# nihui/realsr-ncnn-vulkan

Measured on AMD Instinct MI355X. Metric: output Mpix/s (4x upscale) DF2K tile=200, higher is better.
Workload: dtype f16

## Files before the change

### realsr-ncnn-vulkan_amd/csrc/conv_flow.hip

```cpp
#include "kernels.h"
#include "model.h"

namespace rsr {

typedef _Float16 half8 __attribute__((ext_vector_type(8)));
typedef _Float16 half4 __attribute__((ext_vector_type(4)));
typedef _Float16 half2v __attribute__((ext_vector_type(2)));
typedef float f32x16 __attribute__((ext_vector_type(16)));
typedef unsigned int u32x4 __attribute__((ext_vector_type(4)));
typedef unsigned int u32x2 __attribute__((ext_vector_type(2)));
typedef int i32x8 __attribute__((ext_vector_type(8)));
typedef float f32x4 __attribute__((ext_vector_type(4)));
typedef float f32x2 __attribute__((ext_vector_type(2)));
typedef f32x4 __attribute__((may_alias)) f32x4_lds;

namespace {

constexpr int kFPx = 32;
constexpr int kFRow = kPatchW * kFPx;
constexpr int kFPatch = 20 * 1024;
constexpr int kFPieces = 20;
constexpr int kFItems = kPatchPx * 2;

template <int NT>
struct FlowCfg
{
    static constexpr int PR = NT == 1 ? 6 : 4;
#ifndef RSR_STREAM_WR
#define RSR_STREAM_WR 3
#endif
    static constexpr int WR = RSR_STREAM_WR;
    static constexpr int WB = NT * 9 * 32 * 32;
    static constexpr int WPIECES = NT * 9;
    static constexpr int W_OFF = PR * kFPatch;
    static constexpr int BIAS_OFF = W_OFF + WR * WB;
    static constexpr int TOTAL = BIAS_OFF + NT * 128;
};
static_assert(FlowCfg<1>::TOTAL <= 160 * 1024 && FlowCfg<2>::TOTAL <= 160 * 1024, "LDS budget");

__device__ __forceinline__ const char* plane_ptr(const PlaneSrc& s, int slot, int plane)
{
    return static_cast<const char*>(s.base) + (long long)slot * s.slot_stride + (long long)plane * s.plane_stride;
}

__device__ __forceinline__ WorkItem load_item(const WorkItem* items, int idx)
{
    typedef const __attribute__((address_space(4))) i32x8* cptr_t;
    const i32x8 v = *(cptr_t)(unsigned long long)(items + idx);
    WorkItem it;
    it.slot = __builtin_amdgcn_readfirstlane(v[0]);
    it.y0 = __builtin_amdgcn_readfirstlane(v[1]);
    it.x0 = __builtin_amdgcn_readfirstlane(v[2]);
    it.H = __builtin_amdgcn_readfirstlane(v[3]);
    it.W = __builtin_amdgcn_readfirstlane(v[4]);
    it.pad0 = __builtin_amdgcn_readfirstlane(v[5]);
    it.pad1 = __builtin_amdgcn_readfirstlane(v[6]);
    it.pad2 = __builtin_amdgcn_readfirstlane(v[7]);
    return it;
}

__device__ __forceinline__ char* uniform_ptr(const void* p)
{
    const unsigned long long b = (unsigned long long)p;
    const unsigned lo = (unsigned)__builtin_amdgcn_readfirstlane((int)(unsigned)b);
    const unsigned hi = (unsigned)__builtin_amdgcn_readfirstlane((int)(unsigned)(b >> 32));
    return reinterpret_cast<char*>((unsigned long long)lo | ((unsigned long long)hi << 32));
}

__device__ __forceinline__ f32x2 bf8_pair(unsigned w, int hiword)
{
    return hiword ? __builtin_amdgcn_cvt_pk_f32_bf8(int(w), true) : __builtin_amdgcn_cvt_pk_f32_bf8(int(w), false);
}
__device__ __forceinline__ int pack_bf8_pair(float x, float y, int old, int hiword)
{
    return hiword ? __builtin_amdgcn_cvt_pk_bf8_f32(x, y, old, true) : __builtin_amdgcn_cvt_pk_bf8_f32(x, y, old, false);
}

#define RSR_LDS(p) ((__attribute__((address_space(3))) void*)(p))
#define RSR_GLB(p) ((const __attribute__((address_space(1))) void*)(p))
#define RSR_MFMA 0x8
#define RSR_DSR 0x100
#define RSR_SG(mask, n) __builtin_amdgcn_sched_group_barrier(mask, n, 0)

#ifdef RSR_EXPERIMENT
#define RSR_ABL(bits) (a.dbg & (bits))
#else
#define RSR_ABL(bits) 0
#if defined(RSR_FLOW_LIFE) || defined(RSR_FLOW_TRACE) || defined(RSR_EXP_THIN)
#error "RSR_FLOW_LIFE / RSR_FLOW_TRACE / RSR_EXP_THIN are experiment builds: add -DRSR_EXPERIMENT"
#endif
#endif

}

template <int NT, int NTW, bool UPS, int EPI, bool DEFER, bool WRES>
__global__ __launch_bounds__((4 * NT / NTW + 4) * 64, (4 * NT / NTW + 4) / 4) void conv3x3_flow(const ConvArgs a)
{
    extern __shared__ __attribute__((aligned(16))) char smem[];
    typedef FlowCfg<NT> C;
    constexpr int MW = 4 * NT / NTW;
    constexpr int WB = C::WB;
    constexpr bool WDB = (NTW == 1);
    static_assert(!DEFER || (NT == 1 && NTW == 1), "deferred epilogue needs the 256-VGPR budget of the 8-wave workgroup");
    constexpr bool LAST3 = (EPI == 3 || EPI == 6 || EPI == 8 || EPI == 9);
    constexpr bool LASTG = (EPI == 0 || EPI == 7 || EPI == 10 || EPI == 11);
    constexpr bool OUT32 = (EPI == 6 || EPI == 7 || EPI == 9 || EPI == 11);
    constexpr bool FIMG = EPI >= 8;
    static_assert(!LAST3 || (NT == 1 && NTW == 1 && !UPS && !DEFER && WRES), "conv_last's (dy, cout) layout: 32 rows, resident aux image");
    static_assert((EPI != 4 && EPI != 5) || (NT == 2 && NTW == 1 && !UPS && !DEFER), "the precise residual epilogue exists for the 64-output-channel convs of the trunk");
    constexpr bool RESID = (EPI == 2 || EPI == 4 || EPI == 5);
    constexpr bool PREC = (EPI == 4 || EPI == 5);

    const int tid = threadIdx.x;
    const int lane = tid & 63;
    const int wave = __builtin_amdgcn_readfirstlane(tid >> 6);
#ifdef RSR_FLOW_LIFE
    const unsigned long long life_t0 = __builtin_amdgcn_s_memtime();
#define RSR_LIFE(SLOT) if (a.trace && tid == 0) a.trace[blockIdx.x * 4 + (SLOT)] = __builtin_amdgcn_s_memtime();
#else
#define RSR_LIFE(SLOT)
#endif
    const int nst = a.n0 + a.n1;
    const int PR = WRES ? a.pr : C::PR, WR = WRES ? nst : C::WR;
    const int kWOff = PR * kFPatch, kBiasOff = kWOff + WR * (LAST3 ? a.wpieces * 1024 : WB);

    const int per = (a.nitems + 7) >> 3;
    const int xcd = blockIdx.x & 7, j = blockIdx.x >> 3, nj = gridDim.x >> 3;
    const int first = xcd * per + j;
    const int end = min((xcd + 1) * per, a.nitems);
    const int nmine = first < end ? (end - first + nj - 1) / nj : 0;
    if (nmine == 0) return;
    const int S = nmine * nst;

    if (tid < NT * 32) reinterpret_cast<float*>(smem + kBiasOff)[tid] = a.bias[tid];
    __syncthreads();

    if (wave >= MW)
    {
        const int lw = wave - MW;
        constexpr int NP = kFPieces / 4;
        const int nW = (C::WPIECES - lw + 3) / 4;
        int pr[NP], pc[NP], pxor[NP];
        bool pvalid[NP];
#pragma unroll
        for (int i = 0; i < NP; i++)
        {
            const int jj = (lw + 4 * i) * 64 + lane;
            const int px = jj >> 1;
            pr[i] = px / kPatchW;
            pc[i] = px - pr[i] * kPatchW;
            pxor[i] = ((jj & 1) ^ ((pc[i] >> 3) & 1)) << 4;
            pvalid[i] = jj < kFItems;
        }
        const char* wsrc_lane = static_cast<const char*>(a.wpk16) + lw * 1024 + lane * 16;

        int uP = 0, uW = 0, sP = 0, sW = 0, ckP = 0, ckW = 0, rP = 0;
        WorkItem itP = load_item(a.items, first);
        unsigned srcoff[NP];
        auto block_offsets = [&]() {
            const int H = itP.H, W = itP.W, Wi = UPS ? (W >> 1) : W;
            const bool fold = (itP.x0 & kFoldBit) != 0;
            const int bx0 = itP.x0 & (kFoldBit - 1);
#pragma unroll
            for (int i = 0; i < NP; i++)
            {
                const int half = (fold && pc[i] >= 16) ? 16 : 0;
                const int gy = itP.y0 - 1 + pr[i] + half, gx = bx0 - 1 + pc[i] - half;
                const bool ok = pvalid[i] && gy >= 0 && gy < H && gx >= 0 && gx < W;
                const int sy = UPS ? (gy >> 1) : gy, sx = UPS ? (gx >> 1) : gx;
                srcoff[i] = ok ? unsigned(kGuard + (sy * Wi + sx) * kFPx + pxor[i]) : 0u;
            }
        };
        block_offsets();
        auto issueP = [&]() {
            if (uP >= S) return;
            const char* gbase = ((ckP < a.n0) ? plane_ptr(a.src0, itP.slot, ckP) : plane_ptr(a.src1, itP.slot, ckP - a.n0)) - kGuard;
            char* dst = smem + sP * kFPatch + lw * 1024;
            if (!RSR_ABL(1 | 128))
            {
#pragma unroll
                for (int i = 0; i < NP; i++)
                    __builtin_amdgcn_global_load_lds(RSR_GLB(gbase + srcoff[i]), RSR_LDS(dst + i * 4096), 16, 0, 0);
            }
            sP = sP == PR - 1 ? 0 : sP + 1;
            uP++;
            if (++ckP == nst)
            {
                ckP = 0;
                if (++rP < nmine)
                {
                    itP = load_item(a.items, first + rP * nj);
                    block_offsets();
                }
            }
        };
        auto issueW = [&]() {
            if (uW >= S) return;
            const char* src = wsrc_lane + (long long)ckW * WB;
            char* dst = smem + kWOff + sW * WB + lw * 1024;
            if (!RSR_ABL(1 | 64))
            {
#pragma unroll
                for (int i = 0; i < (C::WPIECES + 3) / 4; i++)
                    if (i < nW)
                        __builtin_amdgcn_global_load_lds(RSR_GLB(src + i * 4096), RSR_LDS(dst + i * 4096), 16, 0, 0);
            }
            sW = sW == WR - 1 ? 0 : sW + 1;
            uW++;
            ckW = ckW + 1 == nst ? 0 : ckW + 1;
        };
        if (WRES)
        {
            const int npieces = nst * (LAST3 ? a.wpieces : C::WPIECES);
            if (!RSR_ABL(1 | 64))
                for (int p_ = lw; p_ < npieces; p_ += 4)
                    __builtin_amdgcn_global_load_lds(RSR_GLB(static_cast<const char*>(a.wpk16) + p_ * 1024 + lane * 16), RSR_LDS(smem + kWOff + p_ * 1024), 16, 0, 0);
            for (int tt = -(PR - 1); tt < 0; tt++) issueP();
            for (int t = 0; t < S; t++)
            {
                if (RSR_ABL(1) || t + PR - 2 >= S) asm volatile("s_waitcnt vmcnt(0)\n\ts_barrier" ::: "memory");
                else if (PR == 3) asm volatile("s_waitcnt vmcnt(%0)\n\ts_barrier" ::"n"(1 * NP) : "memory");
                else if (PR == 4) asm volatile("s_waitcnt vmcnt(%0)\n\ts_barrier" ::"n"(2 * NP) : "memory");
                else if (PR == 5) asm volatile("s_waitcnt vmcnt(%0)\n\ts_barrier" ::"n"(3 * NP) : "memory");
                else if (PR == 6) asm volatile("s_waitcnt vmcnt(%0)\n\ts_barrier" ::"n"(4 * NP) : "memory");
                else asm volatile("s_waitcnt vmcnt(0)\n\ts_barrier" ::: "memory");
                issueP();
            }
        }
        else
        {
            for (int tt = -(PR - 1); tt < 0; tt++)
            {
                if (tt + WR - 1 >= 0) issueW();
                issueP();
            }
            constexpr int WRm2 = C::WR - 2;
            constexpr int NW_HI = (C::WPIECES + 3) / 4, NW_LO = C::WPIECES / 4;
            for (int t = 0; t < S; t++)
            {
                if (RSR_ABL(1) || t + PR - 2 >= S) asm volatile("s_waitcnt vmcnt(0)\n\ts_barrier" ::: "memory");
                else if (RSR_ABL(64)) asm volatile("s_waitcnt vmcnt(%0)\n\ts_barrier" ::"n"((WRm2 + 1) * NP) : "memory");
                else if (RSR_ABL(128) && nW == NW_HI) asm volatile("s_waitcnt vmcnt(%0)\n\ts_barrier" ::"n"(WRm2 * NW_HI) : "memory");
                else if (RSR_ABL(128)) asm volatile("s_waitcnt vmcnt(%0)\n\ts_barrier" ::"n"(WRm2 * NW_LO) : "memory");
                else if (nW == NW_HI) asm volatile("s_waitcnt vmcnt(%0)\n\ts_barrier" ::"n"((WRm2 + 1) * NP + WRm2 * NW_HI) : "memory");
                else asm volatile("s_waitcnt vmcnt(%0)\n\ts_barrier" ::"n"((WRm2 + 1) * NP + WRm2 * NW_LO) : "memory");
                issueW();
                issueP();
            }
        }
        asm volatile("s_barrier" ::: "memory");
        return;
    }

    const int l32 = lane & 31, hi = lane >> 5;
    const int wrow = wave & 3, ntw0 = (wave >> 2) * NTW;
    int xcol[3];
#pragma unroll
    for (int dx = 0; dx < 3; dx++)
    {
        const int c = l32 + dx;
        xcol[dx] = wrow * 4 * kFRow + c * kFPx + ((hi ^ ((c >> 3) & 1)) << 4);
    }
    const int woff = kWOff + (ntw0 * 32 + l32) * 32 + ((hi ^ ((l32 >> 3) & 1)) << 4);

    f32x16 bias16[NTW];
    auto load_bias = [&]() {
#pragma unroll
        for (int n = 0; n < NTW; n++)
#pragma unroll
            for (int q = 0; q < 4; q++)
            {
                const f32x4 b4 = *reinterpret_cast<const f32x4_lds*>(smem + kBiasOff + ((ntw0 + n) * 32 + q * 8 + hi * 4) * 4);
#pragma unroll
                for (int e = 0; e < 4; e++) bias16[n][q * 4 + e] = b4[e];
            }
    };
    load_bias();

    const float slope = a.lrelu ? 0.2f : 1.f;
    const bool idt = RESID && a.res1_in_acc;
    const bool has2 = EPI == 5 || ((EPI == 2) && a.res2_kind == 1);
#ifdef RSR_FLOW_TRACE
    const bool tracing = a.trace && blockIdx.x == 0 && wave == 0;
#else
    constexpr bool tracing = false;
#endif

    float pinf0 = __builtin_inff();
    asm volatile("" : "+s"(pinf0));

    struct OutDesc
    {
        char* base;
        int live;
        int voff;
        int y0, H, W, slot;
        unsigned lim;
    };
    auto make_out = [&](const WorkItem& it, bool live) {
        OutDesc o;
        o.base = const_cast<char*>(plane_ptr(a.out16, it.slot, ntw0 * 2));
        o.live = (live && !RSR_ABL(4)) ? 1 : 0;
        const bool fold = (it.x0 & kFoldBit) != 0;
        const int x = (it.x0 & (kFoldBit - 1)) + (fold ? (l32 & 15) : l32);
        o.voff = x < it.W ? x * kFPx + hi * 16 + ((fold && l32 >= 16) ? 16 * it.W * kFPx : 0) : int(0x80000000u);
        o.y0 = it.y0 + wrow * 4;
        o.H = it.H;
        o.W = it.W;
        o.slot = it.slot;
        o.lim = unsigned(it.H) * unsigned(it.W * kFPx);
        return o;
    };
    auto row_pack = [&](const f32x16& acc, u32x4 (&tq)[2]) {
#pragma unroll
        for (int p = 0; p < 2; p++)
        {
            half8 o;
#pragma unroll
            for (int e = 0; e < 8; e++)
            {
                float v = acc[p * 8 + e];
                if (EPI == 2)
                {
                    v = v * a.s1;
                    asm volatile("" : "+v"(v));
                }
                else v = __builtin_amdgcn_fmed3f(v, v * slope, pinf0);
                o[e] = (_Float16)v;
            }
            tq[p] = __builtin_bit_cast(u32x4, o);
        }
    };
    constexpr bool PRE2 = (EPI == 2 || EPI == 4) && NTW == 1;
    u32x4 r2q[PRE2 ? 2 : 1][NTW][2];
#ifndef RSR_PREC_PRE
#define RSR_PREC_PRE 1
#endif
    u32x4 l1q[EPI == 4 ? 4 : 1];
    auto res2_row = [&](u32x4 (&dst)[2], const OutDesc& o, int rr, int n) {
        const int y = o.y0 + rr;
        char* ub = uniform_ptr(const_cast<char*>(plane_ptr(a.res2, o.slot, ntw0 * 2)));
        const unsigned pstride = unsigned(a.res2.plane_stride);
#pragma unroll
        for (int p = 0; p < 2; p++)
        {
            const unsigned poff = unsigned(n * 2 + p) * pstride;
            const __amdgpu_buffer_rsrc_t rs = __builtin_amdgcn_make_buffer_rsrc(ub, 0, int(o.lim + poff), 0x00020000);
            dst[p] = __builtin_amdgcn_raw_buffer_load_b128(rs, o.voff, int(unsigned(y) * unsigned(o.W * kFPx) + poff), 0);
        }
    };
    auto lo_row = [&](const PlaneSrc& s, long long off, u32x4& dst, const OutDesc& o, int rr, int n) {
        const int y = o.y0 + rr;
        const unsigned pstride = unsigned(s.plane_stride);
        char* ub = uniform_ptr(const_cast<char*>(plane_ptr(s, o.slot, 0)) + off + (long long)(ntw0 + n) * pstride);
        const __amdgpu_buffer_rsrc_t rs = __builtin_amdgcn_make_buffer_rsrc(ub, 0, off ? int(o.lim) : 0, 0x00020000);
        dst = __builtin_amdgcn_raw_buffer_load_b128(rs, o.voff, int(unsigned(y) * unsigned(o.W * kFPx)), 0);
    };
    auto res2_prefetch = [&](const WorkItem& w, int row0) {
        if (!PRE2) return;
        if (EPI == 4)
        {
            if (row0 != 0) return;
            const OutDesc o = make_out(w, true);
#pragma unroll
            for (int rr = 0; rr < RSR_PREC_PRE; rr++) lo_row(a.res1, a.lo1_off, l1q[EPI == 4 ? rr : 0], o, rr, 0);
            __builtin_amdgcn_sched_barrier(0);
            return;
        }
        if (!has2) return;
        const OutDesc o = make_out(w, true);
#pragma unroll
        for (int rr = 0; rr < 2; rr++)
#pragma unroll
            for (int n = 0; n < NTW; n++) res2_row(r2q[PRE2 ? rr : 0][n], o, row0 + rr, n);
        __builtin_amdgcn_sched_barrier(0);
    };
    auto row_store = [&](const u32x4 (&tq)[2], const OutDesc& o, int rr, int n) {
        const int y = o.y0 + rr;
        char* ub = uniform_ptr(o.base);
        const unsigned pstride = unsigned(a.out16.plane_stride);
#pragma unroll
        for (int p = 0; p < 2; p++)
        {
            const unsigned poff = unsigned(n * 2 + p) * pstride;
            const __amdgpu_buffer_rsrc_t rs = __builtin_amdgcn_make_buffer_rsrc(ub, 0, o.live ? int(o.lim + poff) : 0, 0x00020000);
            __builtin_amdgcn_raw_buffer_store_b128(tq[p], rs, o.voff + int(unsigned(y) * unsigned(o.W * kFPx) + poff), 0, 0);
        }
    };
    auto row_emit = [&](const f32x16& acc, const OutDesc& o, int rr, int n) {
        const int y = o.y0 + rr;
        char* ub = uniform_ptr(o.base);
        const unsigned pstride = unsigned(a.out16.plane_stride);
        u32x4 r2x[2];
        if (EPI == 2 && has2 && !PRE2) res2_row(r2x, o, rr, n);
#pragma unroll
        for (int p = 0; p < 2; p++)
        {
            half8 v;
#pragma unroll
            for (int e = 0; e < 8; e++)
            {
                float f = acc[p * 8 + e];
                if (EPI == 2)
                {
                    f = f * a.s1;
                    asm volatile("" : "+v"(f));
                }
                else f = __builtin_amdgcn_fmed3f(f, f * slope, pinf0);
                v[e] = (_Float16)f;
            }
            if (EPI == 2 && has2)
            {
                const half8 r2 = __builtin_bit_cast(half8, PRE2 ? r2q[PRE2 ? (rr & 1) : 0][n][p] : r2x[p]);
#pragma unroll
                for (int e = 0; e < 8; e++)
                {
                    float f = __builtin_fmaf((float)v[e], a.s2, (float)r2[e]);
                    asm volatile("" : "+v"(f));
                    v[e] = (_Float16)f;
                }
            }
            const unsigned poff = unsigned(n * 2 + p) * pstride;
            const __amdgpu_buffer_rsrc_t rs = __builtin_amdgcn_make_buffer_rsrc(ub, 0, o.live ? int(o.lim + poff) : 0, 0x00020000);
            __builtin_amdgcn_raw_buffer_store_b128(__builtin_bit_cast(u32x4, v), rs, o.voff + int(unsigned(y) * unsigned(o.W * kFPx) + poff), 0, 0);
            __builtin_amdgcn_sched_barrier(0);
        }
    };
    constexpr float kLoScale = 2048.f, kLoInv = 1.f / 2048.f;
    auto row_emit4 = [&](const f32x16& acc, const OutDesc& o, int rr, int n, const u32x4& l1, const u32x4 (&r2h)[2], const u32x4& r2l) {
        const int y = o.y0 + rr;
        char* ub = uniform_ptr(o.base);
        const unsigned pstride = unsigned(a.out16.plane_stride);
        char* ul = uniform_ptr(const_cast<char*>(plane_ptr(a.out16, o.slot, 0)) + a.out_lo_off + (long long)(ntw0 + n) * pstride);
        const unsigned rowoff = unsigned(y) * unsigned(o.W * kFPx);
        u32x4 vl;
#pragma unroll
        for (int p = 0; p < 2; p++)
        {
            half8 vh;
            const half8 r = __builtin_bit_cast(half8, r2h[p]);
#pragma unroll
            for (int k = 0; k < 2; k++)
            {
                int wq = 0;
#pragma unroll
                for (int e2 = 0; e2 < 2; e2++)
                {
                    const int c0 = p * 8 + k * 4 + e2 * 2;
                    const f32x2 av = {acc[c0], acc[c0 + 1]};
                    const f32x2 kinv = {kLoInv, kLoInv}, s1v = {a.s1, a.s1};
                    f32x2 f = __builtin_elementwise_fma(bf8_pair(l1[p * 2 + k], e2), kinv, av * s1v);
                    if (EPI == 5)
                    {
                        const f32x2 rv = {(float)r[k * 4 + e2 * 2], (float)r[k * 4 + e2 * 2 + 1]}, s2v = {a.s2, a.s2};
                        f = __builtin_elementwise_fma(bf8_pair(r2l[p * 2 + k], e2), kinv, __builtin_elementwise_fma(f, s2v, rv));
                    }
                    asm volatile("" : "+v"(f));
                    const half2v hv = __builtin_convertvector(f, half2v);
                    vh[k * 4 + e2 * 2] = hv[0];
                    vh[k * 4 + e2 * 2 + 1] = hv[1];
                    const f32x2 ksc = {kLoScale, kLoScale};
                    const f32x2 t = (f - __builtin_convertvector(hv, f32x2)) * ksc;
                    wq = pack_bf8_pair(t[0], t[1], wq, e2);
                }
                vl[p * 2 + k] = unsigned(wq);
            }
            const unsigned poff = unsigned(n * 2 + p) * pstride;
            const __amdgpu_buffer_rsrc_t rs = __builtin_amdgcn_make_buffer_rsrc(ub, 0, o.live ? int(o.lim + poff) : 0, 0x00020000);
            __builtin_amdgcn_raw_buffer_store_b128(__builtin_bit_cast(u32x4, vh), rs, o.voff + int(rowoff + poff), 0, 0);
            __builtin_amdgcn_sched_barrier(0);
        }
        const __amdgpu_buffer_rsrc_t rl = __builtin_amdgcn_make_buffer_rsrc(ul, 0, (o.live && a.out_lo_off) ? int(o.lim) : 0, 0x00020000);
        __builtin_amdgcn_raw_buffer_store_b128(vl, rl, o.voff + int(rowoff), 0, 0);
        __builtin_amdgcn_sched_barrier(0);
    };
    auto store3 = [&](const float (&val)[4][3], const WorkItem& it) {
        if (hi != 0 || ntw0 != 0 || RSR_ABL(4)) return;
        const bool fold = (it.x0 & kFoldBit) != 0;
        const int x = (it.x0 & (kFoldBit - 1)) + (fold ? (l32 & 15) : l32);
        const int yb = it.y0 + wrow * 4 + ((fold && l32 >= 16) ? 16 : 0);
        if (a.out_u8)
        {
            const int ox = it.pad0 + x, ow = pad2_w(it.pad2), oh = pad2_h(it.pad2);
            const int oim = pad2_img(it.pad2);
            uint8_t* const oimg = a.out_u8s[oim];
            const int opitch = a.out_pitch[oim];
            if constexpr (FIMG)
            {
                const long long cstep = a.out_plane[oim];
                const int esh = a.out_fmt == kFmtF32 ? 2 : 1;
#pragma unroll
                for (int rr = 0; rr < 4; rr++)
                {
                    const int y = yb + rr;
                    const int rx = x - a.out_u8_crop, ry = y - a.out_u8_crop;
                    if (rx >= 0 && rx < ow && ry >= 0 && ry < oh)
                    {
                        const long long pix = (long long)(it.pad1 + y) * opitch + ((long long)ox << esh);
#pragma unroll
                        for (int ch = 0; ch < 3; ch++)
                        {
                            float v = OUT32 ? val[rr][ch] : (float)(_Float16)val[rr][ch];
                            v = fminf(fmaxf(v, 0.f), 1.f);
                            uint8_t* const e = oimg + (a.out_u8_bgr ? 2 - ch : ch) * cstep + pix;
                            if (a.out_fmt == kFmtF32) *reinterpret_cast<float*>(e) = v;
                            else *reinterpret_cast<_Float16*>(e) = (_Float16)v;
                        }
                    }
                }
                return;
            }
#pragma unroll
            for (int rr = 0; rr < 4; rr++)
            {
                const int y = yb + rr;
                const int rx = x - a.out_u8_crop, ry = y - a.out_u8_crop;
                if (rx >= 0 && rx < ow && ry >= 0 && ry < oh)
                {
                    uint8_t* o = oimg + (long long)(it.pad1 + y) * opitch + ox * 3;
#pragma unroll
                    for (int ch = 0; ch < 3; ch++)
                    {
                        float v = OUT32 ? val[rr][ch] : (float)(_Float16)val[rr][ch];
                        v = floorf(v * 255.f + 0.5f);
                        v = fminf(fmaxf(v, 0.f), 255.f);
                        o[a.out_u8_bgr ? 2 - ch : ch] = (uint8_t)v;
                    }
                }
            }
            return;
        }
        _Float16* o = reinterpret_cast<_Float16*>(static_cast<char*>(a.out_planar3) + (long long)it.slot * a.planar3_slot_stride);
        const long long hw = (long long)it.H * it.W;
#pragma unroll
        for (int rr = 0; rr < 4; rr++)
        {
            const int y = yb + rr;
            if (y < it.H && x < it.W)
            {
                const long long pix = (long long)y * it.W + x;
#pragma unroll
                for (int ch = 0; ch < 3; ch++)
                {
                    float v = val[rr][ch];
                    if (a.lrelu) v = fmaxf(v, v * 0.2f);
                    if (OUT32) reinterpret_cast<float*>(o)[ch * hw + pix] = v;
                    else o[ch * hw + pix] = (_Float16)v;
                }
            }
        }
    };
    auto planar_store = [&](const f32x16 (&acc)[4][NTW], const WorkItem& it) {
        float val[4][3];
#pragma unroll
        for (int rr = 0; rr < 4; rr++)
#pragma unroll
            for (int ch = 0; ch < 3; ch++) val[rr][ch] = acc[rr][0][ch];
        store3(val, it);
    };

    half8 X[6], Wa[3][NTW], Wb[WDB ? 3 : 1][NTW];
    f32x16 accA[4][NTW], accB[DEFER ? 4 : 1][NTW];

    int sP = 0, sW = 0;
    int r = 0, ck = 0, t = 0;
    auto xbase = [&](int slot, int dx) { return smem + slot * kFPatch + xcol[dx]; };
    auto wbase = [&](int slot) { return smem + slot * WB + woff; };
#define RSR_LDX(R, XB) X[R] = *reinterpret_cast<const half8*>((XB) + (R)*kFRow);
#define RSR_LDW(WS, DY, DX, WBASE)                                                                                   \
    _Pragma("unroll") for (int n_ = 0; n_ < NTW; n_++) WS[DY][n_] =                                                  \
        *reinterpret_cast<const half8*>((WBASE) + ((DY)*3 + (DX)) * (NT * 1024) + n_ * 1024);
#ifndef RSR_EXP_THIN
#define RSR_CELL(ACC, WS, DY, RR, FIRST)                                                                             \
    _Pragma("unroll") for (int n_ = 0; n_ < NTW; n_++) ACC[RR][n_] = __builtin_amdgcn_mfma_f32_32x32x16_f16(         \
        WS[DY][n_], X[(RR) + (DY)], ((FIRST) && (DY) == 0) ? bias16[n_] : ACC[RR][n_], 0, 0, 0);
#else
#define RSR_KEEP(DY, RR)                                                                                             \
    ((DY) == 0 || (RSR_EXP_THIN == 24 && (DY) == 1) ||                                                               \
     (RSR_EXP_THIN == 16 && ((curdx_ == 0 && (DY) == 1 && (RR) == 0) || (curdx_ == 1 && (DY) == 1 && (RR) == 1) || (curdx_ == 2 && (DY) == 2 && (RR) < 2))))
#define RSR_CELL(ACC, WS, DY, RR, FIRST)                                                                             \
    if (RSR_KEEP(DY, RR))                                                                                            \
    {                                                                                                                \
        _Pragma("unroll") for (int n_ = 0; n_ < NTW; n_++) ACC[RR][n_] = __builtin_amdgcn_mfma_f32_32x32x16_f16(     \
            WS[DY][n_], X[(RR) + (DY)], ((FIRST) && (DY) == 0) ? bias16[n_] : ACC[RR][n_], 0, 0, 0);                 \
        if (RSR_EXP_THIN == 16 || ((DY) == 0 && (RR) < 3))                                                           \
        {                                                                                                            \
            half8 y_ = X[((RR) + (DY)) % 6] + X[((RR) + 2 * (DY) + 1) % 6];          \
            if (RSR_EXP_THIN == 16) y_ = y_ + X[((RR) + (DY) + 3) % 6];                                              \
            asm volatile("" ::"v"(y_));                                                                              \
        }                                                                                                            \
    }
#endif
#define RSR_NOHK(c)

#define RSR_STEP(ACC, WCUR, WNXT, NXB, NWB, NDX, FIRST, BAR, ITEMQ, HK)                                              \
    {                                                                                                                \
        constexpr int curdx_ = ((NDX) + 2) % 3;                 \
        (void)curdx_;                                                                                                \
        if ((BAR) && (ITEMQ))                                                                        \
        {                                                                                                            \
            const WorkItem* ip_ = a.items + (first + min(r + 2, nmine - 1) * nj);                                    \
            asm volatile("s_load_dwordx8 %0, %1, 0x0" : "=s"(item_q) : "s"(ip_));                                    \
        }                                                                                                            \
        RSR_CELL(ACC, WCUR, 0, 0, FIRST) HK(0)                                                                       \
        if (!(BAR)) { RSR_LDX(0, NXB) if (WDB) { RSR_LDW(WNXT, 0, NDX, NWB) } }                                      \
        RSR_CELL(ACC, WCUR, 0, 1, FIRST) HK(1) RSR_CELL(ACC, WCUR, 1, 0, FIRST) HK(2)                                \
        if (BAR)                                                                                                     \
        {                                                                                                            \
            __builtin_amdgcn_sched_barrier(0);                                                                       \
            if (tracing) t_arr = __builtin_amdgcn_s_memtime();                                                       \
            if (ITEMQ) asm volatile("s_waitcnt lgkmcnt(0)\n\ts_barrier" : "+s"(item_q)::"memory");                   \
            else asm volatile("s_waitcnt lgkmcnt(0)\n\ts_barrier" ::: "memory");                                     \
            if (tracing) t_rel = __builtin_amdgcn_s_memtime();                                                       \
            __builtin_amdgcn_sched_barrier(0);                                                                       \
            RSR_LDX(0, NXB) if (WDB) { RSR_LDW(WNXT, 0, NDX, NWB) }                                                  \
        }                                                                                                            \
        RSR_LDX(1, NXB) if (WDB) { RSR_LDW(WNXT, 1, NDX, NWB) }                                                      \
        RSR_CELL(ACC, WCUR, 1, 1, FIRST) HK(3) RSR_CELL(ACC, WCUR, 2, 0, FIRST) HK(4) RSR_CELL(ACC, WCUR, 2, 1, FIRST) HK(5) \
        if (WDB) { RSR_LDW(WNXT, 2, NDX, NWB) }                                                                      \
        RSR_CELL(ACC, WCUR, 0, 2, FIRST) HK(6)                                                                       \
        RSR_LDX(2, NXB)                                                                                              \
        RSR_CELL(ACC, WCUR, 0, 3, FIRST) HK(7)                                                                       \
        if (!WDB) { RSR_LDW(WNXT, 0, NDX, NWB) }                                                                     \
        RSR_CELL(ACC, WCUR, 1, 2, FIRST) HK(8)                                                                       \
        RSR_LDX(3, NXB)                                                                                              \
        RSR_CELL(ACC, WCUR, 1, 3, FIRST) HK(9)                                                                       \
        if (!WDB) { RSR_LDW(WNXT, 1, NDX, NWB) }                                                                     \
        RSR_CELL(ACC, WCUR, 2, 2, FIRST) HK(10)                                                                      \
        RSR_LDX(4, NXB)                                                                                              \
        RSR_CELL(ACC, WCUR, 2, 3, FIRST) HK(11)                                                                      \
        RSR_LDX(5, NXB)                                                                                              \
        if (!WDB) { RSR_LDW(WNXT, 2, NDX, NWB) }                                                                     \
    }
#define RSR_STEP_SCHED(BAR, PIN)                                                                                     \
    if (PIN)                                                                                                         \
    {                                                                                                                \
        if (BAR)                                                                                                     \
        {                                                                                                            \
            RSR_SG(RSR_DSR, WDB ? 4 : 2);                                                                            \
            RSR_SG(RSR_MFMA, 3 * NTW);                                                                               \
        }                                                                                                            \
        else                                                                                                         \
        {                                                                                                            \
            RSR_SG(RSR_MFMA, 1 * NTW); RSR_SG(RSR_DSR, WDB ? 2 : 1);                                                 \
            RSR_SG(RSR_MFMA, 2 * NTW); RSR_SG(RSR_DSR, WDB ? 2 : 1);                                                 \
            RSR_SG(RSR_MFMA, 3 * NTW);                                                                               \
        }                                                                                                            \
        if (WDB)                                                                                                     \
        {                                                                                                            \
            RSR_SG(RSR_DSR, 1);                                                                                      \
            RSR_SG(RSR_MFMA, 1); RSR_SG(RSR_DSR, 1);                                                                 \
            RSR_SG(RSR_MFMA, 2); RSR_SG(RSR_DSR, 1);                                                                 \
            RSR_SG(RSR_MFMA, 2); RSR_SG(RSR_DSR, 1);                                                                 \
            RSR_SG(RSR_MFMA, 1); RSR_SG(RSR_DSR, 1);                                                                 \
        }                                                                                                            \
        else                                                                                                         \
        {                                                                                                            \
            RSR_SG(RSR_MFMA, 1 * NTW); RSR_SG(RSR_DSR, 1);                                                           \
            RSR_SG(RSR_MFMA, 1 * NTW); RSR_SG(RSR_DSR, NTW);                                                         \
            RSR_SG(RSR_MFMA, 1 * NTW); RSR_SG(RSR_DSR, 1);                                                           \
            RSR_SG(RSR_MFMA, 1 * NTW); RSR_SG(RSR_DSR, NTW);                                                         \
            RSR_SG(RSR_MFMA, 1 * NTW); RSR_SG(RSR_DSR, 1);                                                           \
            RSR_SG(RSR_MFMA, 1 * NTW); RSR_SG(RSR_DSR, 1 + NTW);                                                     \
        }                                                                                                            \
    }
#define RSR_IDTAP(ACC)                                                                                               \
    if (RESID && idt)                                                                                                \
    {                                                                                                                \
        __builtin_amdgcn_sched_barrier(0);                                                                           \
        _Pragma("unroll") for (int n_ = 0; n_ < NTW; n_++) if ((ck >> 1) == ntw0 + n_)                               \
        {                                                                                                            \
            half8 idf;                                                                                               \
            int l32i = l32;                                                                                          \
            if (PREC) asm volatile("" : "+v"(l32i));  \
            _Pragma("unroll") for (int e = 0; e < 8; e++) idf[e] =                                                   \
                ((ck & 1) * 16 + hi * 8 + e == row_cout(l32i)) ? (_Float16)a.res1_coef : (_Float16)0.f;              \
            const char* cb_ = xbase(sP, 1);                                                                          \
            _Pragma("unroll") for (int rr = 0; rr < 4; rr++)                                                         \
            {                                                                                                        \
                const half8 xc = *reinterpret_cast<const half8*>(cb_ + (rr + 1) * kFRow);                            \
                ACC[rr][n_] = __builtin_amdgcn_mfma_f32_32x32x16_f16(idf, xc, ACC[rr][n_], 0, 0, 0);                 \
            }                                                                                                        \
        }                                                                                                            \
        __builtin_amdgcn_sched_barrier(0);                                                                           \
    }
#define RSR_HALF(ACC, W0, W1, FIRST, HK0, P0, HK1, P1, HK2, P2)                                                      \
    {                                                                                                                \
        const int nsP = sP == PR - 1 ? 0 : sP + 1, nsW = sW == WR - 1 ? 0 : sW + 1;                                  \
        {                                                                                                            \
            const char* nxb = xbase(sP, 1);                                                                          \
            const char* nwb = wbase(sW);                                                                             \
            RSR_STEP(ACC, W0, W1, nxb, nwb, 1, FIRST, false, false, HK0)                                             \
            RSR_STEP_SCHED(false, P0)                                                                                \
        }                                                                                                            \
        RSR_IDTAP(ACC)                                                                                               \
        {                                                                                                            \
            const char* nxb = xbase(sP, 2);                                                                          \
            const char* nwb = wbase(sW);                                                                             \
            RSR_STEP(ACC, W1, W0, nxb, nwb, 2, false, false, false, HK1)                                             \
            RSR_STEP_SCHED(false, P1)                                                                                \
        }                                                                                                            \
        {                                                                                                            \
            const char* nxb = xbase(nsP, 0);                                                                         \
            const char* nwb = wbase(nsW);                                                                            \
            RSR_STEP(ACC, W0, W1, nxb, nwb, 0, false, true, FIRST, HK2)                                              \
            RSR_STEP_SCHED(true, P2)                                                                                 \
        }                                                                                                            \
        if (tracing && lane == 0 && t + 1 < 512)                                                                     \
        {                                                                                                            \
            a.trace[2 * (t + 1)] = t_arr;                                                                            \
            a.trace[2 * (t + 1) + 1] = t_rel;                                                                        \
        }                                                                                                            \
        sP = nsP;                                                                                                    \
        sW = nsW;                                                                                                    \
        t++;                                                                                                         \
    }
#define RSR_HALF_PLAIN(ACC, W0, W1, FIRST) RSR_HALF(ACC, W0, W1, FIRST, RSR_NOHK, 1, RSR_NOHK, 1, RSR_NOHK, 1)

    WorkItem it = load_item(a.items, first);
    WorkItem nxt = load_item(a.items, first + (nmine > 1 ? nj : 0));
    i32x8 item_q = {0, 0, 0, 0, 0, 0, 0, 0};
    auto item_from_q = [&]() {
        WorkItem w;
        w.slot = item_q[0]; w.y0 = item_q[1]; w.x0 = item_q[2]; w.H = item_q[3]; w.W = item_q[4];
        w.pad0 = item_q[5]; w.pad1 = item_q[6]; w.pad2 = item_q[7];
        return w;
    };

    auto wave_is_dead = [&](const WorkItem& w) {
        const int y = w.y0 + wrow * 4;
        return (y >= w.H - a.margin || y + 4 <= a.margin) && !(a.dbg & 32);
    };
    auto skip_block = [&]() {
        {
            const WorkItem* ip_ = a.items + (first + min(r + 2, nmine - 1) * nj);
            asm volatile("s_load_dwordx8 %0, %1, 0x0" : "=s"(item_q) : "s"(ip_));
        }
        for (int h_ = 0; h_ < nst; h_++)
        {
            asm volatile("s_waitcnt lgkmcnt(0)\n\ts_barrier" : "+s"(item_q)::"memory");
            sP = sP == PR - 1 ? 0 : sP + 1;
            sW = sW == WR - 1 ? 0 : sW + 1;
            t++;
        }
        __builtin_amdgcn_sched_barrier(0);
        const char* xb = xbase(sP, 0);
        const char* wb = wbase(sW);
#pragma unroll
        for (int q = 0; q < 6; q++) { RSR_LDX(q, xb) }
#pragma unroll
        for (int dy = 0; dy < 3; dy++) { RSR_LDW(Wa, dy, 0, wb) }
        if (!DEFER) load_bias();
        __builtin_amdgcn_sched_barrier(0);
    };

    unsigned long long t_arr = 0, t_rel = 0;
    (void)t_rel;
    if (tracing) t_arr = __builtin_amdgcn_s_memtime();
    asm volatile("s_barrier" ::: "memory");
#ifdef RSR_FLOW_LIFE
    if (a.trace && tid == 0) a.trace[blockIdx.x * 4 + 0] = life_t0;
    RSR_LIFE(1)
#endif
    if (tracing && lane == 0)
    {
        a.trace[0] = t_arr;
        a.trace[1] = __builtin_amdgcn_s_memtime();
    }
    if constexpr (LAST3)
    {
        f32x16 acc[6];
        half8 Xa[6], Xb[6], Wfa, Wfb;
        const int woff3 = kWOff + l32 * 32 + ((hi ^ ((l32 >> 3) & 1)) << 4);
        const int WB3 = a.wpieces * 1024;
        auto ldx = [&](half8(&Xf)[6], int slot, int dx) {
            const char* xb = xbase(slot, dx);
#pragma unroll
            for (int q = 0; q < 6; q++) Xf[q] = *reinterpret_cast<const half8*>(xb + q * kFRow);
        };
        auto ldw = [&](int plane, int dx) { return *reinterpret_cast<const half8*>(smem + woff3 + plane * WB3 + dx * 1024); };
        const f32x16 zero16 = {0.f, 0.f, 0.f, 0.f, 0.f, 0.f, 0.f, 0.f, 0.f, 0.f, 0.f, 0.f, 0.f, 0.f, 0.f, 0.f};
#define RSR_M6(XF, WF, FIRST)                                                                                        \
    _Pragma("unroll") for (int q = 0; q < 6; q++) acc[q] = __builtin_amdgcn_mfma_f32_32x32x16_f16(WF, XF[q], (FIRST) ? zero16 : acc[q], 0, 0, 0);
#define RSR_HALF3(XC, WC, XN, WN, FIRST)                                                                             \
    {                                                                                                                \
        const int nsP = sP == PR - 1 ? 0 : sP + 1, nck = ck + 1 == nst ? 0 : ck + 1;                                 \
        if (FIRST)  \
        {                                                                                                            \
            const WorkItem* ip_ = a.items + (first + min(r + 2, nmine - 1) * nj);                                    \
            asm volatile("s_load_dwordx8 %0, %1, 0x0" : "=s"(item_q) : "s"(ip_));                                    \
        }                                                                                                            \
        ldx(XN, sP, 1); WN = ldw(ck, 1);                                                                             \
        RSR_M6(XC, WC, FIRST)                                                                                        \
        ldx(XC, sP, 2); WC = ldw(ck, 2);                                                                             \
        RSR_M6(XN, WN, false)                                                                                        \
        __builtin_amdgcn_sched_barrier(0);                                                                           \
        asm volatile("s_waitcnt lgkmcnt(0)\n\ts_barrier" : "+s"(item_q)::"memory");                                  \
        __builtin_amdgcn_sched_barrier(0);                                                                           \
        ldx(XN, nsP, 0); WN = ldw(nck, 0);                                                                           \
        RSR_M6(XC, WC, false)                                                                                        \
        sP = nsP;                                                                                                    \
        t++;                                                                                                         \
    }
        ldx(Xa, 0, 0);
        Wfa = ldw(0, 0);
        for (r = 0; r < nmine; r++)
        {
            while (wave_is_dead(it))
            {
                {
                    const WorkItem* ip_ = a.items + (first + min(r + 2, nmine - 1) * nj);
                    asm volatile("s_load_dwordx8 %0, %1, 0x0" : "=s"(item_q) : "s"(ip_));
                }
                for (int h_ = 0; h_ < nst; h_++)
                {
                    asm volatile("s_waitcnt lgkmcnt(0)\n\ts_barrier" : "+s"(item_q)::"memory");
                    sP = sP == PR - 1 ? 0 : sP + 1;
                    t++;
                }
                ldx(Xa, sP, 0);
                Wfa = ldw(0, 0);
                it = nxt;
                nxt = item_from_q();
                if (++r >= nmine) break;
            }
            if (r >= nmine) break;
            for (int cp = 0; cp < nst; cp += 2)
            {
                ck = cp;
                if (cp == 0) { RSR_HALF3(Xa, Wfa, Xb, Wfb, true) }
                else { RSR_HALF3(Xa, Wfa, Xb, Wfb, false) }
                ck = cp + 1;
                RSR_HALF3(Xb, Wfb, Xa, Wfa, false)
            }
            __builtin_amdgcn_sched_barrier(0);
            float val[4][3];
            const float* bl = reinterpret_cast<const float*>(smem + kBiasOff);
#pragma unroll
            for (int rr = 0; rr < 4; rr++)
#pragma unroll
                for (int ch = 0; ch < 3; ch++) val[rr][ch] = acc[rr][ch] + acc[rr + 1][4 + ch] + acc[rr + 2][8 + ch] + bl[ch];
            store3(val, it);
            __builtin_amdgcn_sched_barrier(0);
            it = nxt;
            nxt = item_from_q();
        }
#undef RSR_HALF3
#undef RSR_M6
        RSR_LIFE(2)
        return;
    }
    {
        const char* xb = xbase(0, 0);
        const char* wb = wbase(0);
#pragma unroll
        for (int rr = 0; rr < 6; rr++) { RSR_LDX(rr, xb) }
#pragma unroll
        for (int dy = 0; dy < 3; dy++) { RSR_LDW(Wa, dy, 0, wb) }
    }

    if (!DEFER)
    {
        for (r = 0; r < nmine; r++)
        {
            while (wave_is_dead(it))
            {
                skip_block();
                it = nxt;
                nxt = item_from_q();
                if (++r >= nmine) break;
            }
            if (r >= nmine) break;
            for (int cp = 0; cp < nst; cp += 2)
            {
                ck = cp;
                if (WDB)
                {
                    if (cp == 0) { RSR_HALF_PLAIN(accA, Wa, Wb, true) }
                    else { RSR_HALF_PLAIN(accA, Wa, Wb, false) }
                    ck = cp + 1;
                    if (cp + 2 >= nst) res2_prefetch(it, 0);
                    RSR_HALF_PLAIN(accA, Wb, Wa, false)
                }
                else
                {
                    if (cp == 0) { RSR_HALF_PLAIN(accA, Wa, Wa, true) }
                    else { RSR_HALF_PLAIN(accA, Wa, Wa, false) }
                    ck = cp + 1;
                    if (PRE2 && cp + 2 >= nst) res2_prefetch(it, 0);
                    RSR_HALF_PLAIN(accA, Wa, Wa, false)
                }
            }
            __builtin_amdgcn_sched_barrier(0);
            auto refill = [&]() {
                __builtin_amdgcn_sched_barrier(0);
                const char* xb = xbase(sP, 0);
                const char* wb = wbase(sW);
#pragma unroll
                for (int q = 0; q < 6; q++) { RSR_LDX(q, xb) }
#pragma unroll
                for (int dy = 0; dy < 3; dy++) { RSR_LDW(Wa, dy, 0, wb) }
                load_bias();
                __builtin_amdgcn_sched_barrier(0);
            };
            if (LASTG)
            {
                planar_store(accA, it);
                refill();
            }
            else if constexpr (PREC && NTW == 1)
            {
                const OutDesc o = make_out(it, true);
                if (EPI == 4)
                {
                    const u32x4 (&nor)[2] = r2q[0][0];
#pragma unroll
                    for (int rr = RSR_PREC_PRE; rr < 4; rr++) lo_row(a.res1, a.lo1_off, l1q[EPI == 4 ? rr : 0], o, rr, 0);
                    __builtin_amdgcn_sched_barrier(0);
#pragma unroll
                    for (int rr = 0; rr < 4; rr++)
                    {
                        if (rr == 3) refill();
                        row_emit4(accA[rr][0], o, rr, 0, l1q[EPI == 4 ? rr : 0], nor, l1q[0]);
                    }
                }
                else
                {
                    u32x4 rh[2][2];
                    u32x4 la[2], ra[2];
#pragma unroll
                    for (int h2 = 0; h2 < 2; h2++)
                    {
#pragma unroll
                        for (int k = 0; k < 2; k++)
                        {
                            res2_row(rh[k], o, 2 * h2 + k, 0);
                            lo_row(a.res1, a.lo1_off, la[k], o, 2 * h2 + k, 0);
                            lo_row(a.res2, a.lo2_off, ra[k], o, 2 * h2 + k, 0);
                        }
                        __builtin_amdgcn_sched_barrier(0);
                        row_emit4(accA[2 * h2][0], o, 2 * h2, 0, la[0], rh[0], ra[0]);
                        if (h2) refill();
                        row_emit4(accA[2 * h2 + 1][0], o, 2 * h2 + 1, 0, la[1], rh[1], ra[1]);
                    }
                }
            }
            else
            {
                const OutDesc o = make_out(it, true);
#pragma unroll
                for (int rr = 0; rr < 4; rr++)
                {
                    if (rr == 3) refill();
#pragma unroll
                    for (int n = 0; n < NTW; n++) row_emit(accA[rr][n], o, rr, n);
                    if (EPI == 2 && rr == 1) res2_prefetch(it, 2);
                }
            }
            __builtin_amdgcn_sched_barrier(0);
            it = nxt;
            nxt = item_from_q();
        }
    }
    else
    {
        OutDesc od = make_out(it, false);
        u32x4 tq[2];
        half2v pk[2][4][2];
        float pinf = __builtin_inff();
        asm volatile("" : "+s"(pinf));
        auto row_store1 = [&](const u32x4& v, const OutDesc& o, int rr, int p) {
            const int y = o.y0 + rr;
            char* ub = uniform_ptr(o.base);
            const unsigned poff = unsigned(p) * unsigned(a.out16.plane_stride);
            const __amdgpu_buffer_rsrc_t rs = __builtin_amdgcn_make_buffer_rsrc(ub, 0, o.live ? int(o.lim + poff) : 0, 0x00020000);
            __builtin_amdgcn_raw_buffer_store_b128(v, rs, o.voff + int(unsigned(y) * unsigned(o.W * kFPx) + poff), 0, 0);
        };
#include "conv_flow_hooks.inc"
#define RSR_BLOCK(ACC)                                                                                               \
    if (wave_is_dead(it))                                                                                            \
    {                                                                                                                \
        if (od.live)                                                                                                 \
        {                                                                                                            \
            _Pragma("unroll") for (int rr = 0; rr < 4; rr++)                                                         \
            {                                                                                                        \
                row_pack(RSR_OLD[rr][0], tq);                                                                        \
                row_store(tq, od, rr, 0);                                                                            \
            }                                                                                                        \
        }                                                                                                            \
        skip_block();                                                                                                \
        _Pragma("unroll") for (int rr = 0; rr < 4; rr++) asm volatile("" : "=v"(ACC[rr][0]));                        \
        od = make_out(it, false);                                                                                    \
        it = nxt;                                                                                                    \
        nxt = item_from_q();                                                                                         \
    }                                                                                                                \
    else                                                                                                             \
    {                                                                                                                \
        ck = 0;                                                                                                      \
        RSR_HALF(ACC, Wa, Wb, true, RSR_HK_S0, RSR_PIN_S0, RSR_HK_S1, RSR_PIN_S1, RSR_HK_S2, RSR_PIN_S2)             \
        ck = 1;                                                                                                      \
        RSR_HALF(ACC, Wb, Wa, false, RSR_HK_S3, RSR_PIN_S3, RSR_HK_S4, RSR_PIN_S4, RSR_HK_S5, RSR_PIN_S5)            \
        ck = 2;                                                                                                      \
        RSR_HALF(ACC, Wa, Wb, false, RSR_HK_S6, RSR_PIN_S6, RSR_HK_S7, RSR_PIN_S7, RSR_HK_S8, RSR_PIN_S8)            \
        ck = 3;                                                                                                      \
        RSR_HALF(ACC, Wb, Wa, false, RSR_HK_S9, RSR_PIN_S9, RSR_HK_S10, RSR_PIN_S10, RSR_HK_S11, RSR_PIN_S11)        \
        for (int cp = 4; cp < nst; cp += 2)                                                                          \
        {                                                                                                            \
            ck = cp;                                                                                                 \
            RSR_HALF_PLAIN(ACC, Wa, Wb, false)                                                                       \
            ck = cp + 1;                                                                                             \
            RSR_HALF_PLAIN(ACC, Wb, Wa, false)                                                                       \
        }                                                                                                            \
        od = make_out(it, true);                                                                                     \
        it = nxt;                                                                                                    \
        nxt = item_from_q();                                                                                         \
    }
        for (r = 0; r < nmine; r += 2)
        {
#define RSR_OLD accB
            RSR_BLOCK(accA)
#undef RSR_OLD
            if (r + 1 < nmine)
            {
                r++;
#define RSR_OLD accA
                RSR_BLOCK(accB)
#undef RSR_OLD
                r--;
            }
        }
        __builtin_amdgcn_sched_barrier(0);
        if (nmine & 1)
        {
#pragma unroll
            for (int rr = 0; rr < 4; rr++)
            {
                row_pack(accA[rr][0], tq);
                row_store(tq, od, rr, 0);
            }
        }
        else
        {
#pragma unroll
            for (int rr = 0; rr < 4; rr++)
            {
                row_pack(accB[rr][0], tq);
                row_store(tq, od, rr, 0);
            }
        }
#undef RSR_BLOCK
#include "conv_flow_hooks_undef.inc"
    }
    RSR_LIFE(2)
#undef RSR_LIFE
#undef RSR_HALF_PLAIN
#undef RSR_HALF
#undef RSR_IDTAP
#undef RSR_STEP
#undef RSR_STEP_SCHED
#undef RSR_CELL
#undef RSR_LDX
#undef RSR_LDW
#undef RSR_NOHK
}

constexpr int kLdsMax = 160 * 1024;

template <int NT, int NTW, bool UPS, int EPI, bool DEFER>
static hipError_t flow_attr()
{
    hipError_t e = hipFuncSetAttribute(reinterpret_cast<const void*>(&conv3x3_flow<NT, NTW, UPS, EPI, DEFER, false>),
                                       hipFuncAttributeMaxDynamicSharedMemorySize, FlowCfg<NT>::TOTAL);
    if (e == hipSuccess)
        e = hipFuncSetAttribute(reinterpret_cast<const void*>(&conv3x3_flow<NT, NTW, UPS, EPI, DEFER, true>),
                                hipFuncAttributeMaxDynamicSharedMemorySize, kLdsMax);
    return e;
}

template <int NT>
static int resident_ring(int nst, int reserve)
{
    const int rest = kLdsMax - nst * FlowCfg<NT>::WB - reserve - NT * 128;
    const int pr = rest / kFPatch;
    return pr < 3 ? 0 : (pr > 6 ? 6 : pr);
}

template <int NT, int NTW, bool UPS, int EPI, bool DEFER>
static void flow_launch(const ConvArgs& a_in, int ncu, bool resident, int reserve, hipStream_t st)
{
    int grid = ncu & ~7;
    const int per = (a_in.nitems + 7) / 8;
    if (per * 8 < grid) grid = per * 8;
    const int nst = a_in.n0 + a_in.n1;
    const int pr = resident ? resident_ring<NT>(nst, reserve * NT) : 0;
    if (pr)
    {
        ConvArgs a = a_in;
        a.pr = pr;
        const int lds = pr * kFPatch + nst * FlowCfg<NT>::WB + NT * 128;
        hipLaunchKernelGGL((conv3x3_flow<NT, NTW, UPS, EPI, DEFER, true>), dim3(grid), dim3((4 * NT / NTW + 4) * 64), lds, st, a);
    }
    else
        hipLaunchKernelGGL((conv3x3_flow<NT, NTW, UPS, EPI, DEFER, false>), dim3(grid), dim3((4 * NT / NTW + 4) * 64), FlowCfg<NT>::TOTAL, st, a_in);
}

#define RSR_FLOW_VARIANTS(F)                                                                                         \
    F(1, 1, false, 0, false) F(1, 1, false, 1, false) F(1, 1, false, 1, true) F(1, 1, false, 2, false) F(1, 1, false, 7, false) \
    F(1, 1, false, 10, false) F(1, 1, false, 11, false)                                                              \
    F(1, 1, true, 1, false)                                                                                          \
    F(2, 1, false, 1, false) F(2, 1, false, 2, false) F(2, 1, true, 1, false) F(2, 1, false, 4, false) F(2, 1, false, 5, false) \
    F(2, 2, false, 1, false) F(2, 2, false, 2, false) F(2, 2, true, 1, false)

hipError_t flow_init_device()
{
    hipError_t e = hipFuncSetAttribute(reinterpret_cast<const void*>(&conv3x3_flow<1, 1, false, 3, false, true>),
                                       hipFuncAttributeMaxDynamicSharedMemorySize, kLdsMax);
    if (e == hipSuccess)
        e = hipFuncSetAttribute(reinterpret_cast<const void*>(&conv3x3_flow<1, 1, false, 6, false, true>), hipFuncAttributeMaxDynamicSharedMemorySize, kLdsMax);
    if (e == hipSuccess)
        e = hipFuncSetAttribute(reinterpret_cast<const void*>(&conv3x3_flow<1, 1, false, 8, false, true>), hipFuncAttributeMaxDynamicSharedMemorySize, kLdsMax);
    if (e == hipSuccess)
        e = hipFuncSetAttribute(reinterpret_cast<const void*>(&conv3x3_flow<1, 1, false, 9, false, true>), hipFuncAttributeMaxDynamicSharedMemorySize, kLdsMax);
#define RSR_F(NT, NTW, UPS, EPI, DEFER)                                                                              \
    if (e == hipSuccess) e = flow_attr<NT, NTW, UPS, EPI, DEFER>();
    RSR_FLOW_VARIANTS(RSR_F)
#undef RSR_F
    return e;
}

bool launch_conv_flow(const ConvArgs& a_in, int nt, int ncu, int flags, hipStream_t st)
{
    if (a_in.nitems <= 0) return true;
    ConvArgs a = a_in;
    if (a.res1_kind == 1 && !a.res1_in_acc)
    {
        if (a.res2_kind) return false;
        a.res2 = a.res1;
        a.lo2_off = a.lo1_off;
        a.lo1_off = 0;
        a.res2_kind = 1;
        a.s2 = 1.f;
    }
    if (((a.n0 + a.n1) & 1) || !a.wpk16) return false;
    const bool ups = a.lvl_out != a.lvl_in;
    int epi = 0;
    if (a.out16.base && !a.out_planar3 && !a.out_u8)
    {
        if (a.res1_kind == 0 && a.res2_kind == 0) epi = 1;
        else if (a.res1_kind == 1 && (a.res2_kind == 0 || a.res2_kind == 1)) epi = 2;
        else return false;
        if (a.precise && (epi == 2 || (epi == 1 && a.out_lo_off && !a.lrelu && !ups))) epi = a.res2_kind ? 5 : 4;
        if (epi >= 4 && !a.res1_kind) a.res1 = a.out16;
    }
    else if ((!a.out_planar3 && !a.out_u8) || a.out16.base || a.res1_kind || a.res2_kind) return false;
    const bool ntw2 = (flags & 1) != 0, defer = !(flags & 2) && a.n0 + a.n1 >= 4, res = !(flags & 4);
    const int reserve = (flags & 16) ? 8192 : 0;
    if (nt == 1)
    {
        if (epi == 0 && !ups && a.waux && !(flags & 8))
        {
            const int nst = a.n0 + a.n1;
            int pr = (kLdsMax - nst * 3072 - 128) / kFPatch;
            pr = pr > 6 ? 6 : pr;
            if (pr < 3) return false;
            a.wpk16 = a.waux;
            a.wpieces = 3;
            a.pr = pr;
            int grid = ncu & ~7;
            const int per = (a.nitems + 7) / 8;
            if (per * 8 < grid) grid = per * 8;
            const bool fimg = a.out_u8 && a.out_fmt != kFmtU8;
            if (fimg && a.precise) hipLaunchKernelGGL((conv3x3_flow<1, 1, false, 9, false, true>), dim3(grid), dim3(512), pr * kFPatch + nst * 3072 + 128, st, a);
            else if (fimg) hipLaunchKernelGGL((conv3x3_flow<1, 1, false, 8, false, true>), dim3(grid), dim3(512), pr * kFPatch + nst * 3072 + 128, st, a);
            else if (a.precise) hipLaunchKernelGGL((conv3x3_flow<1, 1, false, 6, false, true>), dim3(grid), dim3(512), pr * kFPatch + nst * 3072 + 128, st, a);
            else hipLaunchKernelGGL((conv3x3_flow<1, 1, false, 3, false, true>), dim3(grid), dim3(512), pr * kFPatch + nst * 3072 + 128, st, a);
        }
        else if (epi == 0 && !ups && a.out_u8 && a.out_fmt != kFmtU8 && a.precise) flow_launch<1, 1, false, 11, false>(a, ncu, res, reserve, st);
        else if (epi == 0 && !ups && a.out_u8 && a.out_fmt != kFmtU8) flow_launch<1, 1, false, 10, false>(a, ncu, res, reserve, st);
        else if (epi == 0 && !ups && a.precise) flow_launch<1, 1, false, 7, false>(a, ncu, res, reserve, st);
        else if (epi == 0 && !ups) flow_launch<1, 1, false, 0, false>(a, ncu, res, reserve, st);
        else if (epi == 1 && !ups && defer) flow_launch<1, 1, false, 1, true>(a, ncu, res, reserve, st);
        else if (epi == 1 && !ups) flow_launch<1, 1, false, 1, false>(a, ncu, res, reserve, st);
        else if (epi == 1) flow_launch<1, 1, true, 1, false>(a, ncu, res, reserve, st);
        else if (epi == 2 && !ups) flow_launch<1, 1, false, 2, false>(a, ncu, res, reserve, st);
        else return false;
        return true;
    }
    if (nt != 2 || epi == 0) return false;
    if (ntw2 && epi < 4)
    {
        if (epi == 1 && !ups) flow_launch<2, 2, false, 1, false>(a, ncu, res, reserve, st);
        else if (epi == 1) flow_launch<2, 2, true, 1, false>(a, ncu, res, reserve, st);
        else if (epi == 2 && !ups) flow_launch<2, 2, false, 2, false>(a, ncu, res, reserve, st);
        else return false;
    }
    else
    {
        if (epi == 1 && !ups) flow_launch<2, 1, false, 1, false>(a, ncu, res, reserve, st);
        else if (epi == 1) flow_launch<2, 1, true, 1, false>(a, ncu, res, reserve, st);
        else if (epi == 4 && !ups) flow_launch<2, 1, false, 4, false>(a, ncu, res, reserve, st);
        else if (epi == 5 && !ups) flow_launch<2, 1, false, 5, false>(a, ncu, res, reserve, st);
        else if (epi == 2 && !ups) flow_launch<2, 1, false, 2, false>(a, ncu, res, reserve, st);
        else return false;
    }
    return true;
}

}
```

Before: 365.6.

## Stage low-resolution source patch for upsampling convs instead of pre-expanded patch

For the nearest-upsample conv variants, the loader waves now copy only the low-resolution source patch (about a quarter of the pixels, 8 pieces instead of 20) into LDS. The compute waves map each output row and column to its source texel through u_row/u_col when reading X fragments. This cuts global-to-LDS traffic and LDS footprint per patch, which can allow a deeper resident ring. In exchange it adds index arithmetic, and the duplicated-column reads may cause LDS bank conflicts or edge-handling mistakes with folded tiles.

```diff
diff --git a/realsr-ncnn-vulkan_amd/csrc/conv_flow.hip b/realsr-ncnn-vulkan_amd/csrc/conv_flow.hip
--- a/realsr-ncnn-vulkan_amd/csrc/conv_flow.hip
+++ b/realsr-ncnn-vulkan_amd/csrc/conv_flow.hip
@@ -21,6 +21,16 @@
 constexpr int kFPatch = 20 * 1024;
 constexpr int kFPieces = 20;
 constexpr int kFItems = kPatchPx * 2;
+
+constexpr int kUCols = 19, kURows = kBlkH / 2 + 2;
+constexpr int kURow = kUCols * kFPx;
+constexpr int kUItems = kURows * kUCols * 2;
+constexpr int kUPieces = 8;
+constexpr int kUPatch = kUPieces * 1024;
+constexpr __host__ __device__ int u_row(int q) { return (q + 1) >> 1; }
+constexpr __host__ __device__ int u_col(int c) { return ((c + 1) >> 1) + (c >= 16 ? 1 : 0); }
+template <bool UPS>
+constexpr int patch_bytes() { return UPS ? kUPatch : kFPatch; }
 
 template <int NT>
 struct FlowCfg
@@ -122,7 +132,8 @@
 #endif
     const int nst = a.n0 + a.n1;
     const int PR = WRES ? a.pr : C::PR, WR = WRES ? nst : C::WR;
-    const int kWOff = PR * kFPatch, kBiasOff = kWOff + WR * (LAST3 ? a.wpieces * 1024 : WB);
+    constexpr int PB = patch_bytes<UPS>();
+    const int kWOff = PR * PB, kBiasOff = kWOff + WR * (LAST3 ? a.wpieces * 1024 : WB);
 
     const int per = (a.nitems + 7) >> 3;
     const int xcd = blockIdx.x & 7, j = blockIdx.x >> 3, nj = gridDim.x >> 3;
@@ -138,7 +149,7 @@
     if (wave >= MW)
     {
         const int lw = wave - MW;
-        constexpr int NP = kFPieces / 4;
+        constexpr int NP = (UPS ? kUPieces : kFPieces) / 4;
         const int nW = (C::WPIECES - lw + 3) / 4;
         int pr[NP], pc[NP], pxor[NP];
         bool pvalid[NP];
@@ -147,10 +158,10 @@
         {
             const int jj = (lw + 4 * i) * 64 + lane;
             const int px = jj >> 1;
-            pr[i] = px / kPatchW;
-            pc[i] = px - pr[i] * kPatchW;
+            pr[i] = px / (UPS ? kUCols : kPatchW);
+            pc[i] = px - pr[i] * (UPS ? kUCols : kPatchW);
             pxor[i] = ((jj & 1) ^ ((pc[i] >> 3) & 1)) << 4;
-            pvalid[i] = jj < kFItems;
+            pvalid[i] = jj < (UPS ? kUItems : kFItems);
         }
         const char* wsrc_lane = static_cast<const char*>(a.wpk16) + lw * 1024 + lane * 16;
 
@@ -161,6 +172,19 @@
             const int H = itP.H, W = itP.W, Wi = UPS ? (W >> 1) : W;
             const bool fold = (itP.x0 & kFoldBit) != 0;
             const int bx0 = itP.x0 & (kFoldBit - 1);
+            if constexpr (UPS)
+            {
+                const int Hi = H >> 1, sy0 = (itP.y0 >> 1) - 1, sx0 = (bx0 >> 1) - 1;
+#pragma unroll
+                for (int i = 0; i < NP; i++)
+                {
+                    const bool second = pc[i] >= 9;
+                    const int sy = sy0 + pr[i] + ((fold && second) ? 8 : 0), sx = sx0 + pc[i] - (second ? (fold ? 9 : 1) : 0);
+                    const bool ok = pvalid[i] && sy >= 0 && sy < Hi && sx >= 0 && sx < Wi;
+                    srcoff[i] = ok ? unsigned(kGuard + (sy * Wi + sx) * kFPx + pxor[i]) : 0u;
+                }
+                return;
+            }
 #pragma unroll
             for (int i = 0; i < NP; i++)
             {
@@ -175,7 +199,7 @@
         auto issueP = [&]() {
             if (uP >= S) return;
             const char* gbase = ((ckP < a.n0) ? plane_ptr(a.src0, itP.slot, ckP) : plane_ptr(a.src1, itP.slot, ckP - a.n0)) - kGuard;
-            char* dst = smem + sP * kFPatch + lw * 1024;
+            char* dst = smem + sP * PB + lw * 1024;
             if (!RSR_ABL(1 | 128))
             {
 #pragma unroll
@@ -258,8 +282,8 @@
 #pragma unroll
     for (int dx = 0; dx < 3; dx++)
     {
-        const int c = l32 + dx;
-        xcol[dx] = wrow * 4 * kFRow + c * kFPx + ((hi ^ ((c >> 3) & 1)) << 4);
+        const int c = UPS ? u_col(l32 + dx) : l32 + dx;
+        xcol[dx] = (UPS ? wrow * 2 * kURow : wrow * 4 * kFRow) + c * kFPx + ((hi ^ ((c >> 3) & 1)) << 4);
     }
     const int woff = kWOff + (ntw0 * 32 + l32) * 32 + ((hi ^ ((l32 >> 3) & 1)) << 4);
 
@@ -564,9 +588,9 @@
 
     int sP = 0, sW = 0;
     int r = 0, ck = 0, t = 0;
-    auto xbase = [&](int slot, int dx) { return smem + slot * kFPatch + xcol[dx]; };
+    auto xbase = [&](int slot, int dx) { return smem + slot * PB + xcol[dx]; };
     auto wbase = [&](int slot) { return smem + slot * WB + woff; };
-#define RSR_LDX(R, XB) X[R] = *reinterpret_cast<const half8*>((XB) + (R)*kFRow);
+#define RSR_LDX(R, XB) X[R] = *reinterpret_cast<const half8*>((XB) + (UPS ? u_row(R) * kURow : (R)*kFRow));
 #define RSR_LDW(WS, DY, DX, WBASE)                                                                                   \
     _Pragma("unroll") for (int n_ = 0; n_ < NTW; n_++) WS[DY][n_] =                                                  \
         *reinterpret_cast<const half8*>((WBASE) + ((DY)*3 + (DX)) * (NT * 1024) + n_ * 1024);
@@ -1078,10 +1102,10 @@
 }
 
 template <int NT>
-static int resident_ring(int nst, int reserve)
+static int resident_ring(int nst, int reserve, int patch)
 {
     const int rest = kLdsMax - nst * FlowCfg<NT>::WB - reserve - NT * 128;
-    const int pr = rest / kFPatch;
+    const int pr = rest / patch;
     return pr < 3 ? 0 : (pr > 6 ? 6 : pr);
 }
 
@@ -1092,12 +1116,12 @@
     const int per = (a_in.nitems + 7) / 8;
     if (per * 8 < grid) grid = per * 8;
     const int nst = a_in.n0 + a_in.n1;
-    const int pr = resident ? resident_ring<NT>(nst, reserve * NT) : 0;
+    const int pr = resident ? resident_ring<NT>(nst, reserve * NT, patch_bytes<UPS>()) : 0;
     if (pr)
     {
         ConvArgs a = a_in;
         a.pr = pr;
-        const int lds = pr * kFPatch + nst * FlowCfg<NT>::WB + NT * 128;
+        const int lds = pr * patch_bytes<UPS>() + nst * FlowCfg<NT>::WB + NT * 128;
         hipLaunchKernelGGL((conv3x3_flow<NT, NTW, UPS, EPI, DEFER, true>), dim3(grid), dim3((4 * NT / NTW + 4) * 64), lds, st, a);
     }
     else
```

Measured after the change: 366.6 (median of 6 runs). About the same (+0.3%).
